# aharmat/mcptam

Hardware: AMD Instinct MI355X
Metric: ChainBundle LM iters/sec (4-cam, 200 MKF, 50k pts, 400k meas) @1/2/4/8 GPU (higher is better)
Workload: dtype f64; 1 GPU; metric: 4 cams, 200 MKF, 50000 points, 400000 measurements per rank; parallelism=points sharded x1, poses replicated, allreduce_transport=none

## Files before the change

### include/mcp_ba.h

```cpp
#ifndef MCP_BA_H
#define MCP_BA_H

#include <stddef.h>

#ifdef __cplusplus
extern "C" {
#endif

#define MCP_MAX_CHAIN 8
#define MCP_MAX_INV   31

typedef struct mcp_camera {
  double params[9];
  double image_size[2];
  double affine[4];
  double center[2];
  double min_theta;
  double max_rho;
  double theta_mean;
  double theta_std;
  int    n_inv;
  int    pad_;
  double inv_coeffs[MCP_MAX_INV];
} mcp_camera;

typedef struct mcp_ba_params {
  int    max_iterations;
  int    max_trials_after_failure;
  double update_percent_limit;
  double update_rms_limit;
  double min_mestimator_sigma;
  int    disable_convergence;
  int    device;
  int    profile;
} mcp_ba_params;

typedef struct mcp_ba mcp_ba;

typedef struct mcp_ba_iter_log {
  double chi2_start, chi2_end, lambda_end, sigma_sq, rms_update;
  int trials, accepted;
} mcp_ba_iter_log;

typedef struct mcp_ba_timing {
  double total_ms;
  double structure_ms;
  double eval_ms, select_ms, linearize_ms, schur_ms, cholesky_ms, solve_ms, update_ms;
  int    n_linearize, n_trials;
  int    n_solves;
  int    n_spec_hits;
  int    n_collectives_main, n_collectives_spec;
  double collective_bytes_main, collective_bytes_spec;
  int    n_median_fast;
  int    n_persist_fallbacks;
  double schur_mfma_per_system, schur_flops_structural;
  double chol_flops_plan;
  int    chol_chains;
} mcp_ba_timing;

const char* mcp_last_error(void);
int mcp_device_count(void);

mcp_ba* mcp_ba_create(const mcp_camera* cams, int ncam, int use_robust, int use_tukey,
                      int verbose, const mcp_ba_params* params);
void    mcp_ba_destroy(mcp_ba*);

int mcp_ba_add_pose(mcp_ba*, const double R[9], const double t[3], int fixed);
int mcp_ba_add_point(mcp_ba*, const double x[3], const int* chain, int n, int fixed);
int mcp_ba_add_meas(mcp_ba*, const int* chain, int n, int point_id, const double uv[2],
                    double sigma_sq, int cam_index);
int mcp_ba_add_points(mcp_ba*, int count, const double* x , const int* chains,
                      int stride, const int* chain_len, const unsigned char* fixed, int* ids_out);
int mcp_ba_add_measurements(mcp_ba*, int count, const int* chains, int stride,
                            const int* chain_len, const int* point_ids, const double* uv ,
                            const double* sigma_sq, const int* cam_index);

#define MCP_BA_ERR_RUNTIME (-2)
#define MCP_BA_MAX_FREE_POSES 1024
int mcp_ba_compute(mcp_ba*, volatile unsigned char* abort_flag, int n_iter, double user_lambda);

int    mcp_ba_converged(mcp_ba*);
int    mcp_ba_total_iterations(mcp_ba*);
int    mcp_ba_get_point(mcp_ba*, int id, double x[3]);
int    mcp_ba_get_pose(mcp_ba*, int id, double R[9], double t[3]);
int    mcp_ba_get_points(mcp_ba*, int count, const int* ids, double* x);
int    mcp_ba_get_poses(mcp_ba*, int count, const int* ids, double* R, double* t);
int    mcp_ba_num_outliers(mcp_ba*);
int    mcp_ba_get_outliers(mcp_ba*, int* out, int cap);
double mcp_ba_sigma_squared(mcp_ba*);
double mcp_ba_mean_chi_squared(mcp_ba*);
double mcp_ba_max_cov(mcp_ba*);
double mcp_ba_lambda(mcp_ba*);

int    mcp_ba_num_iter_logs(mcp_ba*);
int    mcp_ba_get_iter_logs(mcp_ba*, mcp_ba_iter_log* out, int cap);
int    mcp_ba_get_timing(mcp_ba*, mcp_ba_timing* out);

typedef int (*mcp_allreduce_fn)(void* user, void* device_buf, size_t count, void* hip_stream);
int mcp_ba_set_allreduce(mcp_ba*, mcp_allreduce_fn hook, void* user, int rank, int world_size);

#define MCP_COMM_ID_BYTES 128
typedef struct mcp_comm mcp_comm;
int       mcp_comm_unique_id(void* id_out);
mcp_comm* mcp_comm_init(const void* id, int rank, int world_size, int device);
void      mcp_comm_destroy(mcp_comm*);
int       mcp_ba_set_comm(mcp_ba*, mcp_comm*);
int       mcp_comm_allreduce(mcp_comm*, void* device_buf, size_t count);
int       mcp_comm_allreduce_lane(mcp_comm*, void* device_buf, size_t count, int lane);

int mcp_ba_prepare(mcp_ba*);
// ... 81 lines not shown
```

### mcptam_amd/chain_bundle.py

```python
import ctypes
import os
import time

import numpy as np

from .taylor_camera import camera_array

_HERE = os.path.dirname(os.path.abspath(__file__))
LIB_PATH = os.environ.get("MCP_HIP_LIB") or os.path.join(_HERE, "libmcptam_hip.so")
_LIB = None

c_double_p = ctypes.POINTER(ctypes.c_double)
c_int_p = ctypes.POINTER(ctypes.c_int)
c_ubyte_p = ctypes.POINTER(ctypes.c_ubyte)


class McpBaParams(ctypes.Structure):
    _fields_ = [("max_iterations", ctypes.c_int), ("max_trials_after_failure", ctypes.c_int),
                ("update_percent_limit", ctypes.c_double), ("update_rms_limit", ctypes.c_double),
                ("min_mestimator_sigma", ctypes.c_double), ("disable_convergence", ctypes.c_int),
                ("device", ctypes.c_int), ("profile", ctypes.c_int)]


class McpBaIterLog(ctypes.Structure):
    _fields_ = [("chi2_start", ctypes.c_double), ("chi2_end", ctypes.c_double), ("lambda_end", ctypes.c_double),
                ("sigma_sq", ctypes.c_double), ("rms_update", ctypes.c_double), ("trials", ctypes.c_int),
                ("accepted", ctypes.c_int)]


class McpBaTiming(ctypes.Structure):
    _fields_ = [("total_ms", ctypes.c_double), ("structure_ms", ctypes.c_double), ("eval_ms", ctypes.c_double),
                ("select_ms", ctypes.c_double), ("linearize_ms", ctypes.c_double), ("schur_ms", ctypes.c_double),
                ("cholesky_ms", ctypes.c_double), ("solve_ms", ctypes.c_double), ("update_ms", ctypes.c_double),
                ("n_linearize", ctypes.c_int), ("n_trials", ctypes.c_int), ("n_solves", ctypes.c_int),
                ("n_spec_hits", ctypes.c_int),
                ("n_collectives_main", ctypes.c_int), ("n_collectives_spec", ctypes.c_int),
                ("collective_bytes_main", ctypes.c_double), ("collective_bytes_spec", ctypes.c_double),
                ("n_median_fast", ctypes.c_int), ("n_persist_fallbacks", ctypes.c_int),
                ("schur_mfma_per_system", ctypes.c_double), ("schur_flops_structural", ctypes.c_double),
                ("chol_flops_plan", ctypes.c_double), ("chol_chains", ctypes.c_int)]


class McpBaStructure(ctypes.Structure):
    _fields_ = [(f, ctypes.c_int) for f in (
        "ngroup", "grp_pts", "nbig", "nfl", "np", "grp_points_max", "grp_points_min", "grp_poses_max", "grp_no_pose",
        "grp_blk_max", "grp_inc_max", "lin_kernel", "lin_generic", "schur_kernel", "asm_long", "max_systems", "asm_kernel")]


class McpBaHeadReport(ctypes.Structure):
    _fields_ = [("rank", ctypes.c_ulonglong), ("median", ctypes.c_double), ("sigma", ctypes.c_double * 4),
                ("robust_chi2", ctypes.c_double), ("robust_chi2_plain", ctypes.c_double), ("route_sigma", ctypes.c_double * 4),
                ("head_status", ctypes.c_int), ("overflow", ctypes.c_int), ("pred_ok", ctypes.c_int),
                ("select_overflow", ctypes.c_int), ("n_median_fast", ctypes.c_int), ("declined", ctypes.c_int)]


class McpBaTrialReport(ctypes.Structure):
    _fields_ = [(f, ctypes.c_double) for f in ("robust_chi2", "scale_pose", "scale_point", "scale", "ss_pose", "ss_point", "ss")] + \
               [(f, ctypes.c_int) for f in ("ncb", "nbb", "nchain", "npose", "npoint", "nfl", "np", "nmeas", "small_mode", "given_step")]


HEAD_ROUTES = ("plain", "ranks", "ride", "small", "ahead", "large")
LIN_KERNEL_NAMES = ("none", "quad", "pipe", "group")
SCHUR_KERNEL_NAMES = ("none", "schur4", "schur_group")
ASM_KERNEL_NAMES = ("none", "pair", "tiles", "long")

ALLREDUCE_FN = ctypes.CFUNCTYPE(ctypes.c_int, ctypes.c_void_p, ctypes.c_void_p, ctypes.c_size_t, ctypes.c_void_p)

BA_SYMBOLS = [
    "mcp_last_error", "mcp_device_count", "mcp_ba_create", "mcp_ba_destroy", "mcp_ba_add_pose", "mcp_ba_add_point",
    "mcp_ba_add_meas", "mcp_ba_add_points", "mcp_ba_add_measurements", "mcp_ba_compute", "mcp_ba_converged",
    "mcp_ba_total_iterations", "mcp_ba_get_point", "mcp_ba_get_pose", "mcp_ba_get_points", "mcp_ba_get_poses",
    "mcp_ba_num_outliers", "mcp_ba_get_outliers", "mcp_ba_sigma_squared", "mcp_ba_mean_chi_squared", "mcp_ba_max_cov",
    "mcp_ba_lambda", "mcp_ba_num_iter_logs", "mcp_ba_get_iter_logs", "mcp_ba_get_timing", "mcp_ba_set_allreduce",
    "mcp_ba_prepare", "mcp_ba_eval", "mcp_ba_robust_chi2", "mcp_ba_debug_solve", "mcp_dense_spd_solve",
    "mcp_dense_spd_stress", "mcp_ba_debug_system", "mcp_ba_debug_systems", "mcp_ba_debug_structure", "mcp_ba_debug_head", "mcp_ba_debug_trial", "mcp_chol_debug_factor", "mcp_chol_time", "mcp_chol_debug_runs", "mcp_debug_pose_cut",
    "mcp_ba_struct_cache_stats", "mcp_ba_struct_cache_near_hits", "mcp_ba_struct_cache_clear",
    "mcp_comm_unique_id", "mcp_comm_init", "mcp_comm_destroy", "mcp_ba_set_comm", "mcp_comm_allreduce", "mcp_comm_allreduce_lane",
]


def lib():
    global _LIB
    if _LIB is not None:
        return _LIB
    if not os.path.exists(LIB_PATH):
        raise RuntimeError("libmcptam_hip.so is not built (run `python -c 'import __graft_entry__ as g; g.build()'`); "
                           "the HIP path has no CPU fallback")
    L = ctypes.CDLL(LIB_PATH)
    L.mcp_last_error.restype = ctypes.c_char_p
    L.mcp_ba_create.restype = ctypes.c_void_p
    L.mcp_ba_create.argtypes = [ctypes.c_void_p, ctypes.c_int, ctypes.c_int, ctypes.c_int, ctypes.c_int, ctypes.c_void_p]
    L.mcp_ba_destroy.argtypes = [ctypes.c_void_p]
    L.mcp_ba_add_pose.argtypes = [ctypes.c_void_p, c_double_p, c_double_p, ctypes.c_int]
# ... 433 lines not shown
```

### mcptam_amd/csrc/ba_kernels.h

```cpp
#pragma once
#include "ba_device.h"
#include "ba_select.h"

namespace mcp {

struct DevProblem {
  const mcp_camera* cams; int ncam;
  int nchain;
  const int* chain_len;
  const int* chain_pose;
  int npose;
  const int* pose_unk;
  int npoint;
  const int* pt_chain;
  const int* pt_unk;
  const unsigned char* pt_fixed;
  int nmeas;
  const int* m_pt; const int* m_chain; const unsigned char* m_cam; const unsigned short* m_mask;
  const double* m_u; const double* m_v; const double* m_omega;
  const int* slot_start;
  const int* slot_unk;
  const int* slot_inc;
  int nfl, ninc, np;
  const int* l_i0;
// ... 90 lines not shown
  __syncthreads();
  return t;
}

__device__ inline void robustify(double e2, double s2, double s, double& rho0, double& rho1) {
  if (e2 <= s2) { rho0 = fabs(e2); rho1 = 1.0; }
  else { const double e = sqrt(e2); rho0 = 2.0*s*e - s2; rho1 = s/e; }
}

constexpr int EVAL_BLOCK = 256;

template <bool SUM>
__device__ __forceinline__ void eval_body(const DevProblem& P, const double* __restrict__ pt_x, const double* __restrict__ last,
       double* __restrict__ chi2, double* __restrict__ err_out, const double* __restrict__ sigma,
       double* __restrict__ partial) {
  __shared__ double lds[EVAL_BLOCK/64];
  const int m = blockIdx.x*EVAL_BLOCK + threadIdx.x;
  double contrib = 0.0;
  if (m < P.nmeas) {
    const int pt = P.m_pt[m];
    Se3 Ts, To;
    load_se3(last + 12*(size_t)P.pt_chain[pt], Ts);
    load_se3(last + 12*(size_t)P.m_chain[m], To);
    const double x[3] = { pt_x[3*(size_t)pt], pt_x[3*(size_t)pt+1], pt_x[3*(size_t)pt+2] };
    double xw[3], xc[3];
    se3_apply_inv(Ts, x, xw);
    se3_apply(To, xw, xc);
    Projection pr;
    cam_project<false>(P.cams[P.m_cam[m]], xc, pr);
    const double e0 = P.m_u[m] - pr.u, e1 = P.m_v[m] - pr.v;
    double c = P.m_omega[m]*(e0*e0 + e1*e1);
    if (P.pt_fixed[pt] && P.robust) c = -c;
    chi2[m] = c;
    if (err_out) { err_out[2*(size_t)m] = e0; err_out[2*(size_t)m+1] = e1; }
    if (SUM) {
      if (P.robust) { double r0, r1; robustify(c, sigma[1], sigma[2], r0, r1); contrib = r0; }
      else contrib = c;
    }
  }
  if (SUM) {
    const double t = block_sum<EVAL_BLOCK>(contrib, lds);
    if (threadIdx.x == 0) partial[blockIdx.x] = t;
  }
}

template <bool SUM>
__global__ void __launch_bounds__(EVAL_BLOCK)
k_eval(DevProblem P, const double* __restrict__ pt_x, const double* __restrict__ last,
       double* __restrict__ chi2, double* __restrict__ err_out, const double* __restrict__ sigma,
       double* __restrict__ partial) {
  eval_body<SUM>(P, pt_x, last, chi2, err_out, sigma, partial);
}

__global__ void __launch_bounds__(EVAL_BLOCK)
k_robust_sum(int n, int robust, const double* __restrict__ chi2, const double* __restrict__ sigma,
             double* __restrict__ partial) {
  __shared__ double lds[EVAL_BLOCK/64];
  const int m = blockIdx.x*EVAL_BLOCK + threadIdx.x;
  double contrib = 0.0;
  if (m < n) {
    const double c = chi2[m];
    if (robust) { double r0, r1; robustify(c, sigma[1], sigma[2], r0, r1); contrib = r0; }
    else contrib = c;
  }
  const double t = block_sum<EVAL_BLOCK>(contrib, lds);
  if (threadIdx.x == 0) partial[blockIdx.x] = t;
}

constexpr int MAIL_TICKET = 31;
__device__ __forceinline__ void final_sums_body(int n0, const double* p0, int n1, const double* p1, int n2, const double* p2,
             double* __restrict__ out, int off, const int* __restrict__ fail, double* mail, int mail_count, unsigned long long ticket,
             const double* ride_src, int ride_dst, const double* start_src = nullptr ) {
  __shared__ double lds[4];
  const double* ps[3] = { p0, p1, p2 }; const int ns[3] = { n0, n1, n2 };
  for (int a = 0; a < 3; ++a) {
    if (!ps[a]) continue;
    double v = 0.0;
    for (int i = threadIdx.x; i < ns[a]; i += 256) v += ps[a][i];
    const double t = block_sum<256>(v, lds);
    if (threadIdx.x == 0) out[off + a] = t;
  }
  if (fail && threadIdx.x == 0) out[off + 3] = (fail[0] & 4) ? 1e9 : ((fail[0] != 0) ? 1.0 : 0.0);
  if (ride_src && threadIdx.x == 0) out[ride_dst] = ride_src[0];
  if (mail) {
    __syncthreads();
    for (int i = threadIdx.x; i < mail_count; i += 256) mail[i] = (start_src && i >= 24 && i < 29) ? start_src[i - 24] : out[i];
    __threadfence_system();
    __syncthreads();
    if (threadIdx.x == 0) __hip_atomic_store((unsigned long long*)(mail + MAIL_TICKET), ticket, __ATOMIC_RELEASE, __HIP_MEMORY_SCOPE_SYSTEM);
  }
}
__global__ void __launch_bounds__(256)
k_final_sums(int n0, const double* p0, int n1, const double* p1, int n2, const double* p2,
             double* __restrict__ out, int off, const int* __restrict__ fail, double* mail = nullptr, int mail_count = 0, unsigned long long ticket = 0,
             const double* ride_src = nullptr, int ride_dst = 0 ,
             const double* start_src = nullptr ) {
  final_sums_body(n0, p0, n1, p1, n2, p2, out, off, fail, mail, mail_count, ticket, ride_src, ride_dst, start_src);
}

struct SlotGeom { double B[6]; double base[3]; double sign; };

__device__ inline void slot_jacobian(const SlotGeom& s, double* J ) {
  const double* B = s.B; const double* p = s.base; const double sg = s.sign;
  J[0] = sg*B[0]; J[1] = sg*B[1]; J[2] = sg*B[2];
  J[6] = sg*B[3]; J[7] = sg*B[4]; J[8] = sg*B[5];
  J[3]  = sg*(-B[1]*p[2] + B[2]*p[1]);  J[9]  = sg*(-B[4]*p[2] + B[5]*p[1]);
  J[4]  = sg*( B[0]*p[2] - B[2]*p[0]);  J[10] = sg*( B[3]*p[2] - B[5]*p[0]);
  J[5]  = sg*(-B[0]*p[1] + B[1]*p[0]);  J[11] = sg*(-B[3]*p[1] + B[4]*p[0]);
}

__device__ inline void make_slot(int side, int link, const double* A , const double* xw,
                                 const double* first, const double* second, int oc, int sc,
                                 const double* Robs_last, SlotGeom& s) {
  Se3 F;
  if (side == 0) {
    load_se3(first + 12*(size_t)(oc*MAXC+link), F);
    se3_apply(F, xw, s.base);
    const double* R2 = second + 9*(size_t)(oc*MAXC+link);
#pragma unroll
    for (int r = 0; r < 2; ++r)
#pragma unroll
      for (int c = 0; c < 3; ++c) s.B[3*r+c] = A[3*r]*R2[c] + A[3*r+1]*R2[3+c] + A[3*r+2]*R2[6+c];
    s.sign = 1.0;
  } else {
    load_se3(first + 12*(size_t)(sc*MAXC+link), F);
    se3_apply(F, xw, s.base);
    double Rrel[9];
    mat3_mul_t(Robs_last, F.R, Rrel);
#pragma unroll
    for (int r = 0; r < 2; ++r)
#pragma unroll
      for (int c = 0; c < 3; ++c) s.B[3*r+c] = A[3*r]*Rrel[c] + A[3*r+1]*Rrel[3+c] + A[3*r+2]*Rrel[6+c];
    s.sign = -1.0;
  }
}

constexpr int LIN_BLOCK = 128;

__device__ inline void linearize_one(const DevProblem& P, const int m, const double* __restrict__ pt_x, const double* __restrict__ first,
            const double* __restrict__ second, const double* __restrict__ sigma,
            double* __restrict__ U, double* __restrict__ bp, double* __restrict__ V,
            double* __restrict__ g, double* __restrict__ W) {
  const int pt = P.m_pt[m];
  const int oc = P.m_chain[m], sc = P.pt_chain[pt];
  const int olen = P.chain_len[oc], slen = P.chain_len[sc];
  const int mask = P.m_mask[m];
  const int lpt = P.pt_unk[pt];
  if (mask == 0 && lpt < 0) return;
  Se3 Ts, To;
  load_se3(first + 12*(size_t)(sc*MAXC + slen - 1), Ts);
// ... 376 lines not shown
```

### mcptam_amd/csrc/ba_solver.hip

```cpp
#include <hip/hip_runtime.h>
#include <algorithm>
#include <array>
#include <atomic>
#include <memory>
#include <mutex>
#include <sched.h>
#include <thread>
#include <cfloat>
#include <chrono>
#include <cmath>
#include <cstdio>
#include <cstdlib>
#include <cstring>
#include <condition_variable>
#include <functional>
#include <list>
#include <map>
#include <string>
#include <vector>

#include "../../include/mcp_ba.h"
#include "ba_pool.h"
#include "mcp_knobs.h"
#include "ba_kernels.h"
// ... 376 lines not shown
  std::vector<int> id_kind, id_index;
  int next_id = 1;
  bool dirty = true;

  int nfp = 0, nfl = 0, np = 0, nx = 0, ninc = 0, nslot = 0;
  std::vector<int> perm;
  std::vector<int> fl_point, fp_pose;
  double m_total = 0;
  double nfl_total = 0;
  int nx_total() const { return np + 3*(int)nfl_total; }

  DevBuf<char> d_struct;
  DevBuf<mcp_camera> d_cams;
  DevBuf<int> d_chain_len, d_chain_pose, d_pose_unk, d_pt_chain, d_pt_unk, d_m_pt, d_m_chain;
  DevBuf<unsigned char> d_pt_fixed, d_m_cam, d_flags;
  DevBuf<unsigned short> d_m_mask;
  DevBuf<double> d_m_u, d_m_v, d_m_omega;
  DevBuf<int> d_slot_start, d_slot_unk, d_slot_inc, d_l_i0, d_l_i1, d_inc_unk, d_fl_point;
  DevBuf<int> d_sp_pt, d_sp_m, d_sp_i, d_m_sp, d_l_sp, d_g_sp0, d_g_pose, d_red_tiles;
  DevBuf<double> d_pack; int n_red_tiles = 0;
  DevBuf<unsigned char> d_sp_big, d_slot_lp, d_slot_first, d_inc_lp, d_inc_mixed;
  int nsp = 0, ngroup = 0, nbig = 0;
  static constexpr int NSTATE = 1 + MAX_SYS;
  DevBuf<double> d_pose[NSTATE], d_pt[NSTATE], d_first[NSTATE], d_second[NSTATE], d_last[NSTATE], d_chi2[NSTATE];
  int cur = 0, last_tr = 1;
  int cand(int q) const { for (int s_ = 0, k = 0;; ++s_) { if (s_ == cur) continue; if (k == q) return s_; ++k; } }
  struct SpecLane {
    DevBuf<double> xp, xl, p0, p1, p2;
    bool pre_run = false, ahead_enq = false; unsigned long long pre_ticket = 0;
    hipEvent_t ev_tr = nullptr;
    hipEvent_t ev_wf = nullptr;
    hipStream_t st_tr = nullptr;
    hipStream_t tr_stream = nullptr;
    hipEvent_t head_ev = nullptr; bool head_enq = false; int head_state = -1; unsigned long long head_ticket = 0;
    DevBuf<double> trial; DevBuf<SelState> trstate;
    int pred_ok = 0, ovf = 0;
  };
  SpecLane lane[MAX_SYS];
  DevBuf<double> d_ubig;
  DevBuf<double> d_red;
  DevBuf<double> d_stU, d_stb, d_stS, d_str, d_udiag;
  DevBuf<int> d_g_blk0, d_asm_tiles, d_pair_id, d_pr_start, d_blk_dst, d_po_start, d_rhs_dst, d_asm_tasks;
  DevBuf<unsigned char> d_blk_pair;
  int grp_blk_max = 0;
  int head_ahead_for = -1;
  bool head_ahead_want = false; int dbg_head_ahead = 0;
  int head_ahead(int w);
  struct HeadScratch { unsigned int* hist = nullptr; double* vals = nullptr; double* part = nullptr; double* out = nullptr; double* rs = nullptr; };
  HeadScratch hsc[2*MAX_SYS]; DevBuf<double> d_headbuf;
  hipStream_t st_h = nullptr; bool st_h_own = false;
  unsigned long long head_ticket_ctr = 0;
  int head_par = 0, acc_head_q = -1, dbg_head_miss = 0;
  const double* start_blk = nullptr;
  unsigned int* head_hist(int q) { return hsc[head_par*MAX_SYS + q].hist; }
  int enqueue_head(hipStream_t s, int q, int w, bool side);
  int wait_head(int q);
  bool large_heads() const { return hk.large_head_ahead && robust && !multi() && !small_mode() && d_headbuf.p != nullptr; }
  int head_small(int w, bool sum_aside = false);
  int join_sum();
  int sum_aside(); int sum_w = -1; const double* sum_sig = nullptr;
  hipEvent_t ev_head = nullptr, ev_sum = nullptr; bool sum_pending = false;
  DevBuf<double> d_parth;
  bool small_mode_for(int nmeas_, int nchain_) const { return hk.small_on && !multi() && nmeas_ > 0 && nmeas_ <= SMALL_MEAS && nchain_ <= SMALL_CHAINS; }
  bool small_mode() const { return small_mode_for(P.nmeas, P.nchain); }
  int grp_pts = GRP_PTS;
  int group_points(int nsp) const { return (nsp <= pk.small_points) ? LIN_QUAD_PTS : GRP_PTS; }
  int grp_lmax_pol() const { return hk.group_lmax13 ? S4_LMAX : GRP_LMAX; }
  bool fail_clean = false;
  bool sch4_ok = false;
  double schur_mfma = 0, schur_flops = 0;
  std::vector<unsigned char> last_pat;
  std::string launch_err;
  void note_launch(const char* k) { const hipError_t e = hipGetLastError(); if (e != hipSuccess && e != hipErrorNotReady && launch_err.empty()) launch_err = std::string(k) + ": " + hipGetErrorString(e); }
  std::shared_ptr<StructEntry> pending_entry;
  StructKey cache_key, cache_base; bool cache_insert = false;
  int n_masked = 0;
  unsigned long long med_rank() const { return (unsigned long long)n_masked + (unsigned long long)(m_total/2); }
  DevBuf<int> d_m_last;
  DevBuf<int> d_g_order, d_sp_unk;
  bool sch4_order = false;
  bool asm_long = false;
  bool asm_pair = false;
  int n_asm_tasks = 0, n_asm_walk = 0;
  int grp_inc_max = 0;
  size_t nstage = 0;
  int nrhs_rows = 0;
  AsmPlan A;
  DevBuf<double> d_V, d_g, d_W, d_Vinv, d_xl, d_xp_good, d_xl_good, d_err;
  DevBuf<double> d_selvals;
  DevBuf<double> d_seltab;
  DevBuf<double> d_xp_cand;
  DevBuf<double> d_part0, d_part1, d_part2, d_res, d_sigma, d_hist, d_cov;
  static constexpr int MAX_DIAG_PARTS = 256;
  static int max_diag_parts(int np_, int nfl_) { return std::min(MAX_DIAG_PARTS, (std::max(np_, nfl_) + 1023)/1024); }
  DevBuf<unsigned char> d_headl; bool headl_clean = false; int hl_grid = 0;
  bool use_head_large() const { return pk.head_large_on && robust && !multi() && !small_mode() && P.nmeas > 0 && hl_grid > 0 && d_headl.p != nullptr; }
  int head_large(int w, int off, double* sig_copy2);
  bool hist_clean = false;
  static constexpr int N_SIG = 2 + 2*MAX_SYS;
  int sig_idx = 0;
  double* sig_block(int i) { return d_sigma.p + 8*i; }
  double* sig() { return sig_block(sig_idx); }
  void flip_sig() { sig_idx = (sig_idx == 0) ? 1 : 0; }
  DevBuf<SelState> d_selstate;
  DevBuf<int> d_fail;
  static constexpr size_t HRES = 32 + 32*MAX_SYS + 8 + 2*MAX_SYS;
// ... 1904 lines not shown
        if (e != hipErrorNotReady) { set_err(std::string("stream failed while waiting for a trial: ") + hipGetErrorString(e)); return -1; }
        if (std::chrono::duration<double, std::milli>(std::chrono::steady_clock::now() - w0).count() > hk.timeout_ms)
          return watchdog_fail(q ? "the result of a trial evaluated ahead (speculative lane)" : "the result of a trial (main lane)");
      }
    } else {
#if defined(__x86_64__) || defined(__i386__)
      __builtin_ia32_pause();
#elif defined(__aarch64__)
      __asm__ __volatile__("yield");
#endif
    }
  }
  std::memcpy(h_res, box, count*sizeof(double));
  return 0;
}
int mcp_ba::multi_trial_tail(hipStream_t s, int lane, int q, int slot, int nbe, const double* p0, int nbb, const double* p1, const double* p2,
                             const double* pose_parts, int pose_off, bool main_block, double* mail, int mail_count, unsigned long long ticket) {
  SpecLane& L = this->lane[q];
  double* T = L.trial.p;
  HIPCK(hipMemsetAsync(T, 0, TRIAL_LEN*sizeof(double), s));
  const bool ride = robust && hk.sel_ride && m_total > 0;
  if (ride) {
    const int grid = std::max(1, std::min(256, (P.nmeas + SEL_BLOCK*8 - 1)/(SEL_BLOCK*8)));
    hipLaunchKernelGGL(k_select_hist2, dim3(grid), dim3(SEL_BLOCK), 0, s, P.nmeas, (const double*)d_chi2[slot].p, pred_bin, T + TRIAL_HDR);
  }
  const bool rides = main_block && start_rides;
  hipLaunchKernelGGL(k_final_sums, dim3(1), dim3(256), 0, s, nbe, p0, nbb, p1, nbb, p2, T, 0, (const int*)d_fail.p + q, (double*)nullptr, 0, 0ull,
                     rides ? (const double*)(d_res.p + 24) : (const double*)nullptr, 4);
  if (allreduce(T, ride ? TRIAL_LEN : TRIAL_HDR, lane, false, lane ? "trial evaluated ahead: result block + median histograms" : "trial: result block + median histograms")) return -1;
  hipLaunchKernelGGL(k_trial_post, dim3(1), dim3(SEL_BLOCK), 0, s, T, L.trstate.p, (unsigned long long)(m_total/2), pred_bin, (double)pk.sel_cap, ride ? 1 : 0,
                     pose_parts, pose_off, main_block ? (const double*)(d_res.p + 24) : (const double*)nullptr, rides ? 1 : 0,
                     main_block ? d_res.p : (double*)nullptr, mail, mail_count, ticket);
  if (rides) start_rides = false;
  return 0;
}
int mcp_ba::launch_trial_step(const TrialIo& io) {
  hipStream_t s = io.s;
  const int slot = io.slot;
  const int nbb = backsub_blocks(), nbe = (P.nmeas + EVAL_BLOCK - 1)/EVAL_BLOCK;
  const int ncb = io.stale ? 0 : trial_chain_blocks();
  if (io.main_block) tic(ST_UPDATE);
  if (ncb) { hipLaunchKernelGGL(k_trial_apply, dim3(ncb + (nfl ? nbb : 0)), dim3(256), (size_t)P.npose*12*sizeof(double), s, P, ncb, io.lam, io.rhs, io.bp, (const double*)d_pose[cur].p, d_pose[slot].p, io.pose_parts, io.xp,
                                d_first[slot].p, d_second[slot].p, d_last[slot].p, (const double*)d_g.p, (const double*)d_W.p, io.Vinv,
                                (const double*)d_pt[cur].p, d_pt[slot].p, io.xl, io.p1, io.p2); note_launch("k_trial_apply"); }
  else {
    hipLaunchKernelGGL(k_update_poses, dim3(1), dim3(256), 0, s, P, io.lam, io.rhs, io.bp, (const double*)d_pose[cur].p, d_pose[slot].p, io.pose_parts, io.xp);
    if (nfl && io.stale) hipLaunchKernelGGL(k_apply_point_step, dim3((nfl + 255)/256), dim3(256), 0, s, P, (const double*)io.xl, (const double*)d_pt[cur].p, d_pt[slot].p);
    else if (nfl) hipLaunchKernelGGL(k_backsub, dim3(nbb), dim3(BS_BLOCK), 0, s, P, io.lam, io.rhs, (const double*)d_g.p, (const double*)d_W.p,
                                     io.Vinv, (const double*)d_pt[cur].p, d_pt[slot].p, io.xl, io.p1, io.p2);
  }
  if (io.main_block) { toc(); tic(ST_EVAL); }
  if (io.record_wf) HIPCK(hipEventRecord(lane[io.q].ev_wf, s));
  if (P.nchain && !ncb) hipLaunchKernelGGL(k_chains, dim3((P.nchain + 63)/64), dim3(64), 0, s, P, (const double*)d_pose[slot].p, d_first[slot].p, d_second[slot].p, d_last[slot].p);
  if (nbe) hipLaunchKernelGGL((k_eval<true>), dim3(nbe), dim3(EVAL_BLOCK), 0, s, P, (const double*)d_pt[slot].p, (const double*)d_last[slot].p, d_chi2[slot].p, (double*)nullptr,
                              (const double*)sig(), io.p0);
  const double* p1 = (nfl && !io.stale) ? io.p1 : nullptr; const double* p2 = (nfl && !io.stale) ? io.p2 : nullptr;
  const int nbs = p1 ? nbb : 0;
  if (multi() && !io.stale) {
    if (multi_trial_tail(s, io.lane, io.q, slot, nbe, io.p0, nbs, p1, p2, io.pose_parts, io.pose_off, io.main_block, io.mail, io.mail_count, io.ticket)) return -1;
  } else {
    if (io.main_block && join_sum()) return -1;
    hipLaunchKernelGGL(k_final_sums, dim3(1), dim3(256), 0, s, nbe, (const double*)io.p0, nbs, p1, nbs, p2, io.res, 0, io.fail,
                       io.mail, io.mail_count, io.ticket, (const double*)nullptr, 0, io.main_block ? start_blk : (const double*)nullptr);
    if (io.main_block && !nfl) HIPCK(hipMemsetAsync(d_res.p + 1, 0, 2*sizeof(double), s));
  }
  if (io.main_block) toc();
  return 0;
}
int mcp_ba::enqueue_spec_trial(hipStream_t s, int q) {
  SpecLane& L = lane[q];
  L.tr_stream = s;
  const int slot = cand(q);
  double* rhsq = d_red.p + q*red_stride + (size_t)np*np; double* resq = d_res.p + 32 + 8*q;
  const bool with_head = head_ahead_want && !small_mode() && large_heads() && hk.large_head_ahead != 2 && P.nmeas > 0;
  L.pre_ticket = ++mail_ticket;
  const TrialIo io{s, 1, q, slot, batch_lambda[q], rhsq, rhsq + np, d_Vinv.p + q*vinv_stride, L.xp.p, L.xl.p, L.p0.p, L.p1.p, L.p2.p,
                   resq + 4, 4, resq, d_fail.p + q, h_mail_dev + 32*q, multi() ? MAIL_TICKET : 6, L.pre_ticket, false, true, false};
  if (launch_trial_step(io)) return -1;
  HIPCK(hipEventRecord(L.ev_tr, s));
  L.pre_run = true; L.ahead_enq = true;
  if (with_head) { if (enqueue_head(s, q, slot, true)) return -1; }
  return 0;
}
int mcp_ba::cancel_spec_trials() {
  for (int q = 0; q < MAX_SYS; ++q) lane[q].pre_run = false;
  return 0;
}
int mcp_ba::run_ahead(int q) {
  if (!hk.spec_trials || !hk.use_mailbox || prm.profile) return 0;
  if (multi() && hk.overlap_spec != 1) return 0;
  if (!spec_pending && !spec3_pending && q >= spec2_from) {  }
  if (q < spec2_from || q >= batch_n || lane[q].pre_run) return 0;
  if (hk.spec_trials >= 2 && !multi() && lane[q].st_tr && q > spec2_from) {
    hipEvent_t done = (q >= spec3_from) ? ev_spec3 : ev_spec;
    HIPCK(hipStreamWaitEvent(lane[q].st_tr, done, 0));
    return enqueue_spec_trial(lane[q].st_tr, q);
  }
  return enqueue_spec_trial(q >= spec3_from ? st3 : st2, q);
}
int mcp_ba::read_results(int count) {
  HIPCK(hipMemcpyAsync(h_res, d_res.p, count*sizeof(double), hipMemcpyDeviceToHost, st));
  return wait_stream(st, "a result block");
}

int mcp_ba::linearize() {
  mark("lin_wait", st);
  if ((pk.lin_join_full ? join_spec() : join_spec_lin())) return -1;
  mark("lin_go", st);
  spec_ok = false;
  tic(ST_LIN);
  const size_t n2 = (size_t)np*np;
  if (nbig) {
    HIPCK(hipMemsetAsync(d_ubig.p, 0, (n2 + np)*sizeof(double), st));
    if (nfl) {
      HIPCK(hipMemsetAsync(d_V.p, 0, (size_t)nfl*6*sizeof(double), st));
      HIPCK(hipMemsetAsync(d_g.p, 0, (size_t)nfl*3*sizeof(double), st));
// ... 290 lines not shown
  plan.use_persist = false;
  if (plan.persist.test_fail_launch < 0) {
    CpDevice& dv = cp_device(device);
    if (++dv.real_fallbacks >= 2 && !dv.disabled) { dv.disabled = true; fprintf(stderr, "mcptam_hip: device %d: one-launch Cholesky factorisation switched off for this process after %d hand-off time-outs\n", device, dv.real_fallbacks); }
  }
  spec_ok = false;
  if (cancel_spec_trials()) return -1;
  if (join_spec()) return -1;
  HIPCK(hipStreamSynchronize(st));
  if (st2) HIPCK(hipStreamSynchronize(st2));
  HIPCK(hipMemsetAsync(plan.persist.d_err, 0, 2*sizeof(int)*CholPersist::max_sys, st));
  timing.n_persist_fallbacks++;
  return solve_trial(lam, ok2, ni);
}

int mcp_ba::compute(volatile unsigned char* abort_flag, int n_iter, double user_lambda) {
  LmRun R; R.abort_flag = abort_flag; R.n_iter = n_iter; R.user_lambda = user_lambda;
  if (begin_solve(R)) return MCP_ERR_RUNTIME;
  int nCounter = 0;
  if (nx_total() == 0 || m_total == 0) { nCounter = -1; if (P.nmeas) { launch_chains(cur); launch_eval(cur, false, nullptr); } }
  else {
    tic(ST_EVAL); launch_chains(cur); launch_eval(cur, false, nullptr); toc();
    bool ok = true;
    for (int it = 0; it < R.n_iter && !R.terminate() && ok; ++it) {
      LmIter I; I.it = it; std::memset(&I.lg, 0, sizeof I.lg);
      mark("iter", st);
      if (iteration_head(R, I)) return MCP_ERR_RUNTIME;
      if (it == 0 && initial_lambda(R, I)) return MCP_ERR_RUNTIME;
      I.t0 = std::chrono::steady_clock::now();
      do {
        if (run_trial(R, I)) return MCP_ERR_RUNTIME;
      } while (I.rho < 0 && I.qmax < prm.max_trials_after_failure && !R.terminate());
      if (cancel_spec_trials()) return MCP_ERR_RUNTIME;
      ok = !(I.qmax == prm.max_trials_after_failure || I.rho == 0);
      post_iteration(R, I);
      ++nCounter;
    }
  }
  R.t_loop_end = std::chrono::steady_clock::now();
  return end_solve(R, nCounter);
}
int mcp_ba::begin_solve(LmRun& R) {
  R.t_begin = R.t_first_end = std::chrono::steady_clock::now();
  HIPCK(hipSetDevice(device));
  (void)hipGetLastError(); launch_err.clear(); plan.launch_failed = nullptr;
  std::memset(&timing, 0, sizeof timing);
  evs.clear(); ev_used = 0;
  if (R.n_iter < 0) R.n_iter = prm.max_iterations;
  outliers.clear(); logs.clear();
  if (dirty) { if (prepare()) return MCP_ERR_RUNTIME; }
  timing.schur_mfma_per_system = schur_mfma; timing.schur_flops_structural = schur_flops;
  timing.chol_flops_plan = (np > 0 && plan.persist.ok) ? plan.persist.flops : 0.0;
  timing.chol_chains = (np > 0 && plan.persist.ok) ? plan.persist.nseg : 0;
  converged = 0; total_iterations = 0; spec_hot = 0;
  return 0;
}
int mcp_ba::iteration_head(LmRun& R, LmIter& I) {
  const int it = I.it;
  I.head_done = (it > 0 && head_ahead_for == cur);
  head_ahead_for = -1;
  if (I.head_done) { if (robust) flip_sig(); ++dbg_head_ahead; }
  start_blk = nullptr;
  if (it > 0 && large_heads() && acc_head_q >= 0 && lane[acc_head_q].head_enq && lane[acc_head_q].head_state == cur) { if (head_brought_along(I)) return MCP_ERR_RUNTIME; }
  acc_head_q = -1;
  for (int q = 0; q < MAX_SYS; ++q) lane[q].head_enq = false;
  head_par = it & 1;
  head_ahead_want = (small_mode() || large_heads()) && hk.use_mailbox && !prm.profile && it + 1 < R.n_iter;
  if (I.head_done) { }
  else if (small_mode()) { if (head_small(cur)) return MCP_ERR_RUNTIME; }
  else if (use_head_large()) { if (head_large(cur, RS, nullptr)) return MCP_ERR_RUNTIME; }
  else {
    if (robust) { if (median_sigma(cur)) return MCP_ERR_RUNTIME; }
    tic(ST_EVAL);
    if (robust_total(st, cur, sig(), d_part0.p, d_res.p, RS)) return MCP_ERR_RUNTIME;
    toc();
  }
  if (it == 0) { if (allreduce(d_res.p + RS, 1, 0, false, "iteration-start chi2")) return MCP_ERR_RUNTIME; }
  start_rides = (it > 0 && multi());
  if (!I.lin_done) { if (linearize()) return MCP_ERR_RUNTIME; }
  return 0;
}
int mcp_ba::head_brought_along(LmIter& I) {
  const int q = acc_head_q, keep = sig_idx;
  HeadScratch& H = hsc[head_par*MAX_SYS + q];
  HIPCK(hipStreamWaitEvent(st, lane[q].head_ev, 0));
  sig_idx = 2 + head_par*MAX_SYS + q;
  start_rides = false;
  if (linearize()) return MCP_ERR_RUNTIME;
  const int hs = wait_head(q);
  if (hs < 0) return MCP_ERR_RUNTIME;
  if (hs != 1) { sig_idx = keep; ++dbg_head_miss; return 0; }
  start_blk = H.rs;
  hipStream_t ss = (st2 && ev_sum) ? st2 : st;
  if (ss != st) HIPCK(hipStreamWaitEvent(ss, lane[q].head_ev, 0));
  if (robust_total(ss, cur, sig(), H.part, H.rs, 0)) return MCP_ERR_RUNTIME;
  if (ss != st) { HIPCK(hipEventRecord(ev_sum, ss)); sum_pending = true; }
  I.head_done = true; I.lin_done = true; ++dbg_head_ahead;
  return 0;
}
int mcp_ba::initial_lambda(LmRun& R, LmIter& I) {
  if (!(R.user_lambda > 0)) {
    if (np && asm_long) hipLaunchKernelGGL(k_udiag_long, dim3((np*ASML_LPE + 255)/256), dim3(256), 0, st, A, np, (const double*)d_stU.p, (const double*)Ubig(), d_udiag.p);
    else if (np) hipLaunchKernelGGL(k_udiag, dim3((np + 255)/256), dim3(256), 0, st, A, np, (const double*)d_stU.p, (const double*)Ubig(), d_udiag.p);
    if (multi() && np) { if (allreduce(d_udiag.p, np, 0, false, "pose diagonal for the initial lambda")) return MCP_ERR_RUNTIME; }
    const int nbm = max_diag_parts(np, nfl);
    if (nbm > 1) {
      hipLaunchKernelGGL(k_max_diag_part, dim3(nbm), dim3(256), 0, st, np, (const double*)d_udiag.p, 1, nfl, (const double*)d_V.p, d_part1.p);
      hipLaunchKernelGGL(k_max_of, dim3(1), dim3(256), 0, st, nbm, (const double*)d_part1.p, d_res.p + 5);
    } else
      hipLaunchKernelGGL(k_max_diag, dim3(1), dim3(256), 0, st, np, (const double*)d_udiag.p, 1, nfl, (const double*)d_V.p, d_res.p + 5);
  }
  if (read_results(RS + 5)) return MCP_ERR_RUNTIME;
  if (take_start(I)) return MCP_ERR_RUNTIME;
  R.ni = 2;
  if (R.user_lambda > 0) { lambda = R.user_lambda; return 0; }
  double md = h_res[5];
  if (multi()) {
    if (world > 8) { set_err("more than 8 ranks"); return MCP_ERR_RUNTIME; }
    std::vector<double> slots(world, 0.0); slots[rank] = md;
    HIPCK(hipMemcpyAsync(d_res.p + 16, slots.data(), world*sizeof(double), hipMemcpyHostToDevice, st));
    if (allreduce(d_res.p + 16, world, 0, true, "initial lambda")) return MCP_ERR_RUNTIME;
    HIPCK(hipMemcpy(slots.data(), d_res.p + 16, world*sizeof(double), hipMemcpyDeviceToHost));
    for (double v : slots) md = std::max(md, v);
  }
  lambda = 1e-5*md;
  return 0;
}
int mcp_ba::take_start(LmIter& I) {
// ... 691 lines not shown
    sigp = h->sig(); own_off = 24;
  } else if (route == MCP_BA_HEAD_LARGE) {
    if (h->head_large(w, 24, nullptr)) return -1;
    sigp = h->sig(); own_off = 24;
  } else {
    const int q = 0;
    double* slot = h->sig_block(2 + h->head_par*MAX_SYS + q);
    HIPCK(hipMemcpyAsync(slot, r.route_sigma, 4*sizeof(double), hipMemcpyHostToDevice, st));
    HIPCK(hipStreamSynchronize(st));
    if (h->enqueue_head(st, q, w, false)) return -1;
    const int hs = h->wait_head(q);
    h->lane[q].head_enq = false; h->lane[q].head_state = -1;
    if (hs < 0) return -1;
    r.head_status = hs;
    HIPCK(hipMemcpyAsync(r.route_sigma, slot, 4*sizeof(double), hipMemcpyDeviceToHost, st));
    HIPCK(hipStreamSynchronize(st));
    if (hs == 1) { sigp = slot; medp = h->hsc[h->head_par*MAX_SYS + q].out; }
    else { if (h->median_sigma(w)) return -1; sigp = h->sig(); }
  }
  r.n_median_fast = h->timing.n_median_fast - fast0;
  if (h->multi() && r.n_median_fast == 0) r.select_overflow = h->h_res[30] != 0.0;
  if (route == MCP_BA_HEAD_RANKS) r.overflow = r.select_overflow;
  r.declined = (route == MCP_BA_HEAD_AHEAD && r.head_status != 1) || (route == MCP_BA_HEAD_RIDE && r.n_median_fast == 0);
  if (h->robust_total(st, w, sigp, h->d_part0.p, h->d_res.p, 0)) return -1;
  double own = 0.0;
  HIPCK(hipMemcpyAsync(&r.robust_chi2_plain, h->d_res.p, sizeof(double), hipMemcpyDeviceToHost, st));
  if (own_off >= 0) HIPCK(hipMemcpyAsync(&own, h->d_res.p + own_off, sizeof(double), hipMemcpyDeviceToHost, st));
  HIPCK(hipMemcpyAsync(r.sigma, sigp, 4*sizeof(double), hipMemcpyDeviceToHost, st));
  HIPCK(hipMemcpyAsync(&r.median, medp, sizeof(double), hipMemcpyDeviceToHost, st));
  HIPCK(hipStreamSynchronize(st));
  r.robust_chi2 = own_off >= 0 ? own : r.robust_chi2_plain;
  if (route == MCP_BA_HEAD_LARGE) { unsigned long long b; std::memcpy(&b, &own, 8); if (b == HL_FAILED_BITS) { set_err("mcp_ba_debug_head: the head (k_head_large) gave up at a barrier"); return -1; } }
  if (!h->launch_err.empty()) { set_err("mcp_ba_debug_head: launch refused: " + h->launch_err); h->launch_err.clear(); return -1; }
  *out = r;
  return 0;
}

int mcp_ba_debug_trial(mcp_ba* h, double lambda, const double* x, int n_poses, int n_points, int n_meas, double* x_out,
                       double* poses_out, double* points_out, double* chi2_out, mcp_ba_trial_report* out) {
  if (!out) { set_err("mcp_ba_debug_trial: no report block"); return -1; }
  if (h->dirty && h->prepare()) return -1;
  HIPCK(hipSetDevice(h->device));
  if (h->multi()) { set_err("mcp_ba_debug_trial: refused: an all-reduce hook or communicator is installed (the hook runs one rank's trial on the main stream)"); return -1; }
  if (h->P.nmeas == 0 || h->nx == 0) { set_err("mcp_ba_debug_trial: empty problem"); return -1; }
  if (n_poses != (int)h->poses.size() || n_points != (int)h->points.size() || n_meas != (int)h->meas.size()) {
    char msg[224]; snprintf(msg, sizeof msg, "mcp_ba_debug_trial: outputs sized for %d poses, %d points, %d measurements, the handle has %d, %d, %d",
                            n_poses, n_points, n_meas, (int)h->poses.size(), (int)h->points.size(), (int)h->meas.size());
    set_err(msg); return -1;
  }
  hipStream_t st = h->st;
  const int np = h->np, nfl = h->nfl;
  if (h->cancel_spec_trials() || h->join_spec() || h->join_sum()) return -1;
  h->head_ahead_want = false; h->head_ahead_for = -1;
  if (h->state_ready(true)) return -1;
  mcp_ba_trial_report r; std::memset(&r, 0, sizeof r);
  r.ncb = x ? 0 : h->trial_chain_blocks(); r.nbb = nfl ? h->backsub_blocks() : 0;
  r.nchain = h->P.nchain; r.npose = h->P.npose; r.npoint = h->P.npoint; r.nfl = nfl; r.np = np; r.nmeas = (int)h->meas.size();
  r.small_mode = h->small_mode() ? 1 : 0; r.given_step = x ? 1 : 0;
  {
    const int s0 = h->cand(0);
    auto nans = [&](double* p, size_t n) { return (p && n) ? hipMemsetAsync(p, 0xFF, n*sizeof(double), st) : hipSuccess; };
    HIPCK(nans(h->d_first[s0].p, h->d_first[s0].n)); HIPCK(nans(h->d_second[s0].p, h->d_second[s0].n)); HIPCK(nans(h->d_last[s0].p, h->d_last[s0].n));
    HIPCK(nans(h->d_chi2[s0].p, h->d_chi2[s0].n));
    HIPCK(nans(h->d_xp_cand.p, h->d_xp_cand.n)); HIPCK(nans(h->d_xl.p, h->d_xl.n));
    HIPCK(nans(h->d_part0.p, h->d_part0.n)); HIPCK(nans(h->d_part1.p, h->d_part1.n)); HIPCK(nans(h->d_part2.p, h->d_part2.n));
    std::vector<double> ps(h->poses.size()*12), pt(h->points.size()*3);
    if (!ps.empty()) HIPCK(hipMemcpyAsync(ps.data(), h->d_pose[s0].p, ps.size()*8, hipMemcpyDeviceToHost, st));
    if (!pt.empty()) HIPCK(hipMemcpyAsync(pt.data(), h->d_pt[s0].p, pt.size()*8, hipMemcpyDeviceToHost, st));
    HIPCK(hipStreamSynchronize(st));
    for (size_t i = 0; i < h->poses.size(); ++i) if (h->poses[i].unk >= 0) std::memset(&ps[i*12], 0xFF, 96);
    for (size_t i = 0; i < h->points.size(); ++i) if (h->points[i].unk >= 0) std::memset(&pt[i*3], 0xFF, 24);
    if (!ps.empty()) HIPCK(hipMemcpyAsync(h->d_pose[s0].p, ps.data(), ps.size()*8, hipMemcpyHostToDevice, st));
    if (!pt.empty()) HIPCK(hipMemcpyAsync(h->d_pt[s0].p, pt.data(), pt.size()*8, hipMemcpyHostToDevice, st));
    HIPCK(hipStreamSynchronize(st));
  }
  DevBuf<double> gxp, gxl;
  const double* xl_dev = h->d_xl.p;
  int slot;
  if (!x) {
    bool ok2 = true;
    if (h->solve_trial(lambda, ok2)) return -1;
    if (!ok2) { set_err("mcp_ba_debug_trial: system not positive definite"); return -1; }
    slot = h->last_tr;
    r.scale = h->h_res[1]; r.ss = h->h_res[2];
    double raw[8];
    HIPCK(hipMemcpyAsync(raw, h->d_res.p, sizeof raw, hipMemcpyDeviceToHost, st));
    HIPCK(hipStreamSynchronize(st));
    r.robust_chi2 = raw[0];
    r.scale_point = nfl ? raw[1] : 0.0; r.ss_point = nfl ? raw[2] : 0.0;
    r.scale_pose = raw[6]; r.ss_pose = raw[7];
  } else {
    if (gxp.alloc((size_t)np) || gxl.alloc((size_t)nfl*3)) return -1;
    if (np) HIPCK(hipMemcpyAsync(gxp.p, x, (size_t)np*8, hipMemcpyHostToDevice, st));
    if (nfl) HIPCK(hipMemcpyAsync(gxl.p, x + np, (size_t)nfl*24, hipMemcpyHostToDevice, st));
    HIPCK(hipStreamSynchronize(st));
    h->sys_cur = 0; h->spec_ok = false;
    slot = h->cand(0);
    const mcp_ba::TrialIo io{st, 0, h->sys_cur, slot, lambda, gxp.p, h->bp(), nullptr, h->d_xp_cand.p, gxl.p, h->d_part0.p, nullptr, nullptr,
                             h->d_res.p + 6, 6, h->d_res.p, nullptr, nullptr, 0, 0ull, false, false, true};
    if (h->launch_trial_step(io)) return -1;
    if (h->read_results(1)) return -1;
    r.robust_chi2 = h->h_res[0];
    xl_dev = gxl.p;
  }
  const size_t nps = (size_t)h->P.npose*12, npt = (size_t)h->P.npoint*3; const int n = h->P.nmeas;
  std::vector<double> c(chi2_out ? n : 0);
// ... 344 lines not shown
```

Before: 2183 LM iterations/s (x map shards).

## Fold iteration-start robust chi2 sum into first trial eval and final-sums kernels

Result: faster. 2230 LM iterations/s (x map shards), median of 6 (+2.2%).

```diff
diff --git a/include/mcp_ba.h b/include/mcp_ba.h
--- a/include/mcp_ba.h
+++ b/include/mcp_ba.h
@@ -56,6 +56,7 @@
   double schur_mfma_per_system, schur_flops_structural;
   double chol_flops_plan;
   int    chol_chains;
+  int    n_start_rides;
 } mcp_ba_timing;
 
 const char* mcp_last_error(void);
diff --git a/mcptam_amd/chain_bundle.py b/mcptam_amd/chain_bundle.py
--- a/mcptam_amd/chain_bundle.py
+++ b/mcptam_amd/chain_bundle.py
@@ -38,7 +38,7 @@
                 ("collective_bytes_main", ctypes.c_double), ("collective_bytes_spec", ctypes.c_double),
                 ("n_median_fast", ctypes.c_int), ("n_persist_fallbacks", ctypes.c_int),
                 ("schur_mfma_per_system", ctypes.c_double), ("schur_flops_structural", ctypes.c_double),
-                ("chol_flops_plan", ctypes.c_double), ("chol_chains", ctypes.c_int)]
+                ("chol_flops_plan", ctypes.c_double), ("chol_chains", ctypes.c_int), ("n_start_rides", ctypes.c_int)]
 
 
 class McpBaStructure(ctypes.Structure):
diff --git a/mcptam_amd/csrc/ba_kernels.h b/mcptam_amd/csrc/ba_kernels.h
--- a/mcptam_amd/csrc/ba_kernels.h
+++ b/mcptam_amd/csrc/ba_kernels.h
@@ -166,10 +166,7 @@
   eval_body<SUM>(P, pt_x, last, chi2, err_out, sigma, partial);
 }
 
-__global__ void __launch_bounds__(EVAL_BLOCK)
-k_robust_sum(int n, int robust, const double* __restrict__ chi2, const double* __restrict__ sigma,
-             double* __restrict__ partial) {
-  __shared__ double lds[EVAL_BLOCK/64];
+__device__ __forceinline__ double robust_sum_term(int n, int robust, const double* __restrict__ chi2, const double* __restrict__ sigma) {
   const int m = blockIdx.x*EVAL_BLOCK + threadIdx.x;
   double contrib = 0.0;
   if (m < n) {
@@ -177,39 +174,96 @@
     if (robust) { double r0, r1; robustify(c, sigma[1], sigma[2], r0, r1); contrib = r0; }
     else contrib = c;
   }
+  return contrib;
+}
+__device__ __forceinline__ void robust_sum_block(double contrib, double* __restrict__ partial, double* lds) {
   const double t = block_sum<EVAL_BLOCK>(contrib, lds);
   if (threadIdx.x == 0) partial[blockIdx.x] = t;
 }
+__global__ void __launch_bounds__(EVAL_BLOCK)
+k_robust_sum(int n, int robust, const double* __restrict__ chi2, const double* __restrict__ sigma,
+             double* __restrict__ partial) {
+  __shared__ double lds[EVAL_BLOCK/64];
+  robust_sum_block(robust_sum_term(n, robust, chi2, sigma), partial, lds);
+}
+__global__ void __launch_bounds__(EVAL_BLOCK)
+k_eval_start(DevProblem P, const double* __restrict__ pt_x, const double* __restrict__ last,
+             double* __restrict__ chi2, const double* __restrict__ sigma, double* __restrict__ partial,
+             int robust, const double* __restrict__ chi2_cur, double* __restrict__ partial_cur) {
+  __shared__ double lds[EVAL_BLOCK/64];
+  const double start_term = robust_sum_term(P.nmeas, robust, chi2_cur, sigma);
+  eval_body<true>(P, pt_x, last, chi2, nullptr, sigma, partial);
+  robust_sum_block(start_term, partial_cur, lds);
+}
 
 constexpr int MAIL_TICKET = 31;
+constexpr int FS_ARRAYS = 4;
+constexpr int FS_AHEAD = 8;
+static_assert(MAIL_TICKET <= 64, "the forwarded block is one wavefront's: lane i holds entry i");
 __device__ __forceinline__ void final_sums_body(int n0, const double* p0, int n1, const double* p1, int n2, const double* p2,
              double* __restrict__ out, int off, const int* __restrict__ fail, double* mail, int mail_count, unsigned long long ticket,
-             const double* ride_src, int ride_dst, const double* start_src = nullptr ) {
-  __shared__ double lds[4];
-  const double* ps[3] = { p0, p1, p2 }; const int ns[3] = { n0, n1, n2 };
-  for (int a = 0; a < 3; ++a) {
-    if (!ps[a]) continue;
-    double v = 0.0;
-    for (int i = threadIdx.x; i < ns[a]; i += 256) v += ps[a][i];
-    const double t = block_sum<256>(v, lds);
-    if (threadIdx.x == 0) out[off + a] = t;
-  }
-  if (fail && threadIdx.x == 0) out[off + 3] = (fail[0] & 4) ? 1e9 : ((fail[0] != 0) ? 1.0 : 0.0);
-  if (ride_src && threadIdx.x == 0) out[ride_dst] = ride_src[0];
+             const double* ride_src, int ride_dst, const double* start_src = nullptr ,
+             int n3 = 0, const double* p3 = nullptr, int dst3 = 0) {
+  __shared__ double lds[FS_ARRAYS][4];
+  const int t = threadIdx.x;
+  const double* ps[FS_ARRAYS] = { p0, p1, p2, p3 };
+  const int ns[FS_ARRAYS] = { p0 ? n0 : 0, p1 ? n1 : 0, p2 ? n2 : 0, p3 ? n3 : 0 };
+  const bool from_start = start_src && t >= 24 && t < 29;
+  double fw = 0.0;
+  if (mail && t < mail_count) fw = from_start ? start_src[t - 24] : out[t];
+  int zero = 0; asm volatile("" : "+v"(zero));  const int fl = fail ? fail[zero] : 0;
+  const double rd = ride_src ? ride_src[zero] : 0.0;
+  double v[FS_ARRAYS] = { 0.0, 0.0, 0.0, 0.0 };
+  const int nmax = max(max(ns[0], ns[1]), max(ns[2], ns[3]));
+  for (int base = 0; base < nmax; base += 256*FS_AHEAD) {
+    double x[FS_ARRAYS][FS_AHEAD];
+#pragma unroll
+    for (int a = 0; a < FS_ARRAYS; ++a)
+#pragma unroll
+      for (int k = 0; k < FS_AHEAD; ++k) { const int i = base + 256*k + t; x[a][k] = (i < ns[a]) ? ps[a][i] : 0.0; }
+#pragma unroll
+    for (int a = 0; a < FS_ARRAYS; ++a)
+#pragma unroll
+      for (int k = 0; k < FS_AHEAD; ++k) if (base + 256*k + t < ns[a]) v[a] += x[a][k];
+  }
+#pragma unroll
+  for (int a = 0; a < FS_ARRAYS; ++a) {
+#pragma unroll
+    for (int o = 32; o > 0; o >>= 1) v[a] += __shfl_down(v[a], o, 64);
+    if ((t & 63) == 0) lds[a][t >> 6] = v[a];
+  }
+  __syncthreads();
+  if (t < 64) {
+    double tot[FS_ARRAYS];
+#pragma unroll
+    for (int a = 0; a < FS_ARRAYS; ++a) { double s = 0.0; for (int i = 0; i < 4; ++i) s += lds[a][i]; tot[a] = s; }
+    const double fv = (fl & 4) ? 1e9 : ((fl != 0) ? 1.0 : 0.0);
+#pragma unroll
+    for (int a = 0; a < FS_ARRAYS; ++a) {
+      if (!ps[a]) continue;
+      const int d = (a < 3) ? off + a : dst3;
+      if (t == 0) out[d] = tot[a];
+      if (t == d && !from_start) fw = tot[a];
+    }
+    if (fail) { if (t == 0) out[off + 3] = fv; if (t == off + 3 && !from_start) fw = fv; }
+    if (ride_src) { if (t == 0) out[ride_dst] = rd; if (t == ride_dst && !from_start) fw = rd; }
+    if (mail) {
+      if (t < mail_count) mail[t] = fw;
+      __threadfence_system();
+    }
+  }
   if (mail) {
     __syncthreads();
-    for (int i = threadIdx.x; i < mail_count; i += 256) mail[i] = (start_src && i >= 24 && i < 29) ? start_src[i - 24] : out[i];
-    __threadfence_system();
-    __syncthreads();
-    if (threadIdx.x == 0) __hip_atomic_store((unsigned long long*)(mail + MAIL_TICKET), ticket, __ATOMIC_RELEASE, __HIP_MEMORY_SCOPE_SYSTEM);
+    if (t == 0) __hip_atomic_store((unsigned long long*)(mail + MAIL_TICKET), ticket, __ATOMIC_RELEASE, __HIP_MEMORY_SCOPE_SYSTEM);
   }
 }
 __global__ void __launch_bounds__(256)
 k_final_sums(int n0, const double* p0, int n1, const double* p1, int n2, const double* p2,
              double* __restrict__ out, int off, const int* __restrict__ fail, double* mail = nullptr, int mail_count = 0, unsigned long long ticket = 0,
              const double* ride_src = nullptr, int ride_dst = 0 ,
-             const double* start_src = nullptr ) {
-  final_sums_body(n0, p0, n1, p1, n2, p2, out, off, fail, mail, mail_count, ticket, ride_src, ride_dst, start_src);
+             const double* start_src = nullptr ,
+             int n3 = 0, const double* p3 = nullptr, int dst3 = 0 ) {
+  final_sums_body(n0, p0, n1, p1, n2, p2, out, off, fail, mail, mail_count, ticket, ride_src, ride_dst, start_src, n3, p3, dst3);
 }
 
 struct SlotGeom { double B[6]; double base[3]; double sign; };
diff --git a/mcptam_amd/csrc/ba_solver.hip b/mcptam_amd/csrc/ba_solver.hip
--- a/mcptam_amd/csrc/ba_solver.hip
+++ b/mcptam_amd/csrc/ba_solver.hip
@@ -452,6 +452,7 @@
   unsigned long long head_ticket_ctr = 0;
   int head_par = 0, acc_head_q = -1, dbg_head_miss = 0;
   const double* start_blk = nullptr;
+  bool start_ride = false;
   unsigned int* head_hist(int q) { return hsc[head_par*MAX_SYS + q].hist; }
   int enqueue_head(hipStream_t s, int q, int w, bool side);
   int wait_head(int q);
@@ -2462,7 +2463,11 @@
   if (io.main_block) { toc(); tic(ST_EVAL); }
   if (io.record_wf) HIPCK(hipEventRecord(lane[io.q].ev_wf, s));
   if (P.nchain && !ncb) hipLaunchKernelGGL(k_chains, dim3((P.nchain + 63)/64), dim3(64), 0, s, P, (const double*)d_pose[slot].p, d_first[slot].p, d_second[slot].p, d_last[slot].p);
-  if (nbe) hipLaunchKernelGGL((k_eval<true>), dim3(nbe), dim3(EVAL_BLOCK), 0, s, P, (const double*)d_pt[slot].p, (const double*)d_last[slot].p, d_chi2[slot].p, (double*)nullptr,
+  const bool ride = io.main_block && start_ride;
+  if (ride) { start_ride = false; ++timing.n_start_rides; }
+  if (ride) hipLaunchKernelGGL(k_eval_start, dim3(nbe), dim3(EVAL_BLOCK), 0, s, P, (const double*)d_pt[slot].p, (const double*)d_last[slot].p, d_chi2[slot].p,
+                               (const double*)sig(), io.p0, robust ? 1 : 0, (const double*)d_chi2[cur].p, d_parth.p);
+  else if (nbe) hipLaunchKernelGGL((k_eval<true>), dim3(nbe), dim3(EVAL_BLOCK), 0, s, P, (const double*)d_pt[slot].p, (const double*)d_last[slot].p, d_chi2[slot].p, (double*)nullptr,
                               (const double*)sig(), io.p0);
   const double* p1 = (nfl && !io.stale) ? io.p1 : nullptr; const double* p2 = (nfl && !io.stale) ? io.p2 : nullptr;
   const int nbs = p1 ? nbb : 0;
@@ -2470,8 +2475,10 @@
     if (multi_trial_tail(s, io.lane, io.q, slot, nbe, io.p0, nbs, p1, p2, io.pose_parts, io.pose_off, io.main_block, io.mail, io.mail_count, io.ticket)) return -1;
   } else {
     if (io.main_block && join_sum()) return -1;
+    if (io.mail_count > MAIL_TICKET) { set_err("a trial's mailbox block is longer than the mailbox"); return -1; }
     hipLaunchKernelGGL(k_final_sums, dim3(1), dim3(256), 0, s, nbe, (const double*)io.p0, nbs, p1, nbs, p2, io.res, 0, io.fail,
-                       io.mail, io.mail_count, io.ticket, (const double*)nullptr, 0, io.main_block ? start_blk : (const double*)nullptr);
+                       io.mail, io.mail_count, io.ticket, (const double*)nullptr, 0, io.main_block ? start_blk : (const double*)nullptr,
+                       ride ? nbe : 0, ride ? (const double*)d_parth.p : (const double*)nullptr, RS);
     if (io.main_block && !nfl) HIPCK(hipMemsetAsync(d_res.p + 1, 0, 2*sizeof(double), s));
   }
   if (io.main_block) toc();
@@ -2868,7 +2875,7 @@
   timing.schur_mfma_per_system = schur_mfma; timing.schur_flops_structural = schur_flops;
   timing.chol_flops_plan = (np > 0 && plan.persist.ok) ? plan.persist.flops : 0.0;
   timing.chol_chains = (np > 0 && plan.persist.ok) ? plan.persist.nseg : 0;
-  converged = 0; total_iterations = 0; spec_hot = 0;
+  converged = 0; total_iterations = 0; spec_hot = 0; start_ride = false;
   return 0;
 }
 int mcp_ba::iteration_head(LmRun& R, LmIter& I) {
@@ -2876,7 +2883,7 @@
   I.head_done = (it > 0 && head_ahead_for == cur);
   head_ahead_for = -1;
   if (I.head_done) { if (robust) flip_sig(); ++dbg_head_ahead; }
-  start_blk = nullptr;
+  start_blk = nullptr; start_ride = false;
   if (it > 0 && large_heads() && acc_head_q >= 0 && lane[acc_head_q].head_enq && lane[acc_head_q].head_state == cur) { if (head_brought_along(I)) return MCP_ERR_RUNTIME; }
   acc_head_q = -1;
   for (int q = 0; q < MAX_SYS; ++q) lane[q].head_enq = false;
@@ -2887,9 +2894,12 @@
   else if (use_head_large()) { if (head_large(cur, RS, nullptr)) return MCP_ERR_RUNTIME; }
   else {
     if (robust) { if (median_sigma(cur)) return MCP_ERR_RUNTIME; }
-    tic(ST_EVAL);
-    if (robust_total(st, cur, sig(), d_part0.p, d_res.p, RS)) return MCP_ERR_RUNTIME;
-    toc();
+    start_ride = it > 0 && !multi() && hk.use_mailbox && !prm.profile && P.nmeas > 0 && d_parth.p;
+    if (!start_ride) {
+      tic(ST_EVAL);
+      if (robust_total(st, cur, sig(), d_part0.p, d_res.p, RS)) return MCP_ERR_RUNTIME;
+      toc();
+    }
   }
   if (it == 0) { if (allreduce(d_res.p + RS, 1, 0, false, "iteration-start chi2")) return MCP_ERR_RUNTIME; }
   start_rides = (it > 0 && multi());
@@ -3687,6 +3697,7 @@
   const int np = h->np, nfl = h->nfl;
   if (h->cancel_spec_trials() || h->join_spec() || h->join_sum()) return -1;
   h->head_ahead_want = false; h->head_ahead_for = -1;
+  h->start_ride = false;
   if (h->state_ready(true)) return -1;
   mcp_ba_trial_report r; std::memset(&r, 0, sizeof r);
   r.ncb = x ? 0 : h->trial_chain_blocks(); r.nbb = nfl ? h->backsub_blocks() : 0;
```
